# rcelha/rio-rs

Measured on AMD Instinct MI355X. Metric: placement decisions/sec + achieved HBM GB/s, 10M objects x 1 024 nodes, higher is better.
Workload: dtype u32; 1 GPU; config 3: 10000000 objects x 1024 nodes, Zipf(1.1) load, cap 1.25x; a stream of committed ticks that starts from the cold table (all pending); objects_per_gpu=10000000, nodes=1024, parallelism=rows sharded x1

## Files before the change

### include/rio_gpu_placement_debug.h

```cpp
#ifndef RIO_GPU_PLACEMENT_DEBUG_H
#define RIO_GPU_PLACEMENT_DEBUG_H

#include "rio_gpu_placement.h"

#ifdef __cplusplus
extern "C" {
#endif

int rio_gp_debug_set_compact(rio_gp_t* h, int mode);
uint64_t rio_gp_debug_chained_scans(rio_gp_t* h);
int rio_gp_debug_set_speculate(rio_gp_t* h, int speculate);
int rio_gp_debug_set_node_index(rio_gp_t* h, uint32_t tile_rows);
int rio_gp_debug_node_index_geometry(rio_gp_t* h, const uint64_t* node_bitmap, uint32_t* out4);
void rio_gp_debug_set_scan_nt(int mode);
void rio_gp_debug_set_part_shift(int shift);
uint64_t rio_gp_debug_wave_row_lo(uint64_t n_objects, uint32_t n_nodes, uint32_t wave, uint32_t* n_waves);
int rio_gp_debug_ktrace(rio_gp_t* h, int enable, int table, uint64_t* out2048);
int rio_gp_debug_stream_probe(rio_gp_t* h, int mode, int reps, float* ms);

#ifdef __cplusplus
}
#endif
#endif
```

### rio-rs_amd/csrc/placement_kernels.h

```cpp
#pragma once
#include <hip/hip_runtime.h>
#include <stdint.h>

namespace riogp {

typedef uint32_t u32;
typedef unsigned long long u64;

constexpr u32 kNone = 0xFFFFFFFFu;
constexpr u32 kSpillMark = 0xFFFFFFFEu;
constexpr u32 kSkipMark = 0xFFFFFFFDu;
constexpr u32 kAffInactive = 0xFFFFFFFEu;
constexpr u32 kFlagReplaced = 0x10u;
constexpr u32 kNoCut = 0xFFFFFFFFu;

constexpr int kWaves = 16;
constexpr int kBlock = kWaves * 64;
constexpr int kTile = 256;
constexpr u32 kMaxBlocks = 256;
constexpr u32 kMaxSubs = 256;
constexpr int kMidBatch = 16384;
constexpr int kReqBatch = 131072;
constexpr int kSmallBatch = 256;

struct Plan {
    u64 n;
    u64 tiles;
    u64 tq;
    u64 div_magic;
    u32 tr;
    u32 nw;
    u32 G;
    u32 sub;
    u32 subs;
    u32 m;
    u32 mwords;
    u32 trace;
    u32 sa;
    u64 mark;
    const u32* wcnt;
    u32* alive_dst;
};
Plan make_plan(u64 n, u32 m, u32 max_blocks);
// ... 21 lines not shown
    u64* H;
    u64* partial;
    u64* blkstat;
    u64* wsp_sum[2];
    u32* wsp_cnt[2];
    u64* bsp_sum[2];
    u32* bsp_cnt[2];
    u64* used_kept;
    u64* used_cur;
    u64* claim_tot;
    u32* cutblk;
    u64* budget;
    u64* admpre;
    u32* cutidx;
    u32* forced_bits;
    u64* rank_base;
    const u64* pending_global;
    const u64* run_if = nullptr;
    u64* RP;
    u64* R;
    u64* D;
    const u64* used_snap;
    u64* Tg = nullptr;
    DevStats* stats;
    FxRows fx;
};
constexpr u32 kFillRounds = 8;

struct PackOut {
    u32* idx;
    u32* load;
    u32* aff;
    u32* next;
    u32* wcnt;
};

struct Table {
    const u32* cur;
    const u32* load;
    const u32* aff;
    u32* next;
    const u32* pk_idx = nullptr;
    u32* real_next = nullptr;
    bool none_prewritten = false;
    const uint2* vrec = nullptr;
    bool prewritten = false;
// ... 18 lines not shown
    u64* rows = nullptr;
};

bool scan_chain_fits(u32 m);

void launch_scan(const Plan& p, const Table& t, const NodeTab& nt, const SolveBufs& b, bool virt, bool all_alive,
                 hipStream_t s, hipEvent_t e0 = nullptr, hipEvent_t e1 = nullptr, const PackOut* pack = nullptr,
                 const ScanChain* chain = nullptr);
void launch_resolve(const Plan& p, const NodeTab& nt, const SolveBufs& b, u64* host_partial, hipStream_t s,
                    hipEvent_t e0 = nullptr, hipEvent_t e1 = nullptr, const PackOut* search = nullptr,
                    u64* fold_into = nullptr, u32 fold_rounds = 0, const u64* kept_from = nullptr, const u64* fold_from = nullptr);
bool inc_scan_fits(u32 m);
void launch_inc_scan(const Plan& p, u32* assign, const u32* load, const u32* aff, const NodeTab& nt, const SolveBufs& b,
                     const PackOut& pack, hipStream_t s);
Plan rebal_plan(const Plan& p);
u64 rebal_rows(u64 n);
void launch_rebal(const Plan& p, const Plan& pv, const PackOut& src, const NodeTab& nt, const PackOut& dst, const SolveBufs& b,
                  hipStream_t s);
unsigned resolve_blocks(u32 m);
void set_scan_nt(int mode);
void launch_cut_find(const Plan& p, const Table& t, const NodeTab& nt, const SolveBufs& b, bool virt, hipStream_t s,
                     bool have_cutblk);
void launch_fill(const Plan& p, const Table& t, const NodeTab& nt, const SolveBufs& b, bool virt, bool apply, bool fill,
                 int round, bool last, hipStream_t s, const PackOut* pack = nullptr);
bool fill_can_pack(u32 m);
bool cut_apply_fits(u32 m);
void launch_cut_apply(const Plan& p, const Table& t, const NodeTab& nt, const SolveBufs& b, const PackOut& pk, const PackOut& ul,
                      u64* Tg, bool pack, bool all_alive, hipStream_t s);
void launch_used_fold(u64* used, const u64* D, u32 m, u32 rounds, hipStream_t s);
#ifdef RIO_GP_LAB
int ktrace_enable(int on);
int ktrace_read(int table, u64* out );
float sync_probe(int mode, int reps, hipStream_t s);
float stream_probe(int mode, const u32* a, const u32* b, const u32* c, u32* o, u64 n, int reps, hipStream_t s,
                   hipEvent_t e0, hipEvent_t e1);
#endif

struct SmallInline { u32 a[4]; u32 b[4]; };
void launch_lookup_small(const u32* assign, u64 n_obj, const u32* idx, u32 n, u32* out, DevStats* st, hipStream_t s,
                         u32* done, u32 seq, const SmallInline* inl = nullptr);
void launch_lookup(const u32* assign, u64 n_obj, const u32* idx, u64 n, u32* out, DevStats* st, hipStream_t s,
                   u32* done = nullptr, u32 seq = 0, unsigned int* ticket = nullptr);
void launch_update(u32* assign, u64 n_obj, u32 m, const u32* idx, const u32* node, u64 n, u32* pos_scratch,
                   DevStats* st, hipStream_t s, u32* aff_life = nullptr, unsigned int* ticket = nullptr, u32* done = nullptr,
                   u32 seq = 0, u64* used = nullptr, const u32* load = nullptr);
void launch_update_small(u32* assign, const u32* idx, const u32* node, u32 n, hipStream_t s, u32* aff_life = nullptr,
                         u32* done = nullptr, u32 seq = 0, const SmallInline* inl = nullptr, u64* used = nullptr,
// ... 186 lines not shown
```

### rio-rs_amd/csrc/placement_kernels.hip

```cpp
#include "placement_kernels.h"
#include <algorithm>
#include <cstdlib>

#include <hip/hip_ext.h>

namespace riogp {


template <int CTRL>
__device__ __forceinline__ u64 dpp64(u64 v) {
    const u32 lo = (u32)__builtin_amdgcn_update_dpp(0, (int)(u32)v, CTRL, 0xf, 0xf, false);
    const u32 hi = (u32)__builtin_amdgcn_update_dpp(0, (int)(u32)(v >> 32), CTRL, 0xf, 0xf, false);
    return ((u64)hi << 32) | lo;
}
template <int CTRL>
__device__ __forceinline__ u32 dpp32(u32 v) {
    return (u32)__builtin_amdgcn_update_dpp(0, (int)v, CTRL, 0xf, 0xf, false);
}
__device__ __forceinline__ u64 shfl_up64(u64 v, int d) {
    u32 lo = __shfl_up((u32)v, d, 64), hi = __shfl_up((u32)(v >> 32), d, 64);
    return ((u64)hi << 32) | lo;
}
__device__ __forceinline__ u64 shfl_xor64(u64 v, int d) {
    u32 lo = __shfl_xor((u32)v, d, 64), hi = __shfl_xor((u32)(v >> 32), d, 64);
// ... 1723 lines not shown
        rk[q] = 0;
        if (q < per && cls[q] < 0x100u)
            rk[q] = (u32)ctot[cls[q]] + (u32)tab[((size_t)cls[q] * per + q) * kWaves + wave] + pos[q];
    }
    RIOGP_KT(p, 4, 4);
    return all;
}


struct FillArgs {
    const u32* cur; const u32* load; const u32* aff; u32* next;
    const u32* alive_bits;
    Plan p;
    const u32* cutidx; const u32* forced_bits;
    const u64* cap; const u64* Uread; const u64* D; u64* Uadd; u32 round;
    const u64* wsp_sum_in; const u32* wsp_cnt_in; u64* wsp_sum_out; u32* wsp_cnt_out;
    const u64* bsp_sum_in; const u32* bsp_cnt_in; u64* bsp_sum_out; u32* bsp_cnt_out;
    const u64* R; const u64* RP; u32 ng;
    int last;
    DevStats* stats;
    const u32* pk_idx; u32* real_next;
    const u64* rank_base; const u64* pending_global;
    const u64* run_if;
    FxRows fx;
    PackOut pko;
};

__host__ __device__ __forceinline__ size_t fill_lds_x(u32 m, u32 mwords, bool pack) {
    const size_t a = (size_t)m * sizeof(u64);
    const size_t b = (size_t)((m + 3) & ~3u) * sizeof(u32) + (size_t)((mwords + 3) & ~3u) * sizeof(u32) +
                     (pack ? (size_t)kWaves * 2 * kStageCap * sizeof(u32) : 0);
    const size_t c = rank_tab_bytes(m);
    const size_t x = a > b ? a : b;
    return ((x > c ? x : c) + 15) & ~(size_t)15;
}
__host__ __device__ __forceinline__ size_t fill_lds_off_ord(u32 m) { return 512 + (((size_t)(m + 1) * sizeof(u64) + 15) & ~(size_t)15); }
__host__ __device__ __forceinline__ size_t fill_lds_off_x(u32 m) { return fill_lds_off_ord(m) + (((size_t)m * sizeof(unsigned short) + 15) & ~(size_t)15); }

template <bool VIRT, bool APPLY, bool FILL, bool PACK>
__global__ __launch_bounds__(kBlock) void k_fill(const FillArgs a) {
    extern __shared__ __attribute__((aligned(16))) unsigned char smem[];
    const Plan& p = a.p;
    const u32 m = p.m;
    const bool sa_ = p.sa != 0;
    u64* red = reinterpret_cast<u64*>(smem);
    u64* part = reinterpret_cast<u64*>(smem + 128);
// ... 39 lines not shown
    if (FILL) {
#pragma unroll
        for (u32 q = 0; q < 8; ++q) fr[q] = 0;
        pgv = a.pending_global ? *a.pending_global : 0ull;
        rbv = a.rank_base ? *a.rank_base : 0ull;
#pragma unroll
        for (u32 q = 0; q < 8; ++q) {
            if (q < per) {
                const u32 j = tid + q * kBlock, jj = j < m ? j : m - 1;
                u64 u = a.Uread[jj];
                if (a.D)
                    for (u32 r = 0; r < a.round; ++r) u += a.D[(size_t)r * m + jj];
                const u64 c = a.cap[jj];
                const bool al = bit_of(a.alive_bits, jj);
                fr[q] = (j < m && al && c > u) ? c - u : 0ull;
            }
        }
    }
    const u32 bt = (u32)tid < G ? (u32)tid : G - 1;
    const u64 bv = a.bsp_sum_in[bt] + ((APPLY && FILL) ? a.R[bt] : 0ull);
    const u64 rpv = (APPLY && FILL) ? a.RP[(size_t)((u32)tid < a.ng ? (u32)tid : a.ng - 1) * G + blockIdx.x] : 0ull;
    const u32 bc = a.bsp_cnt_in[bt];
    const u64 pw = a.wsp_sum_in[w0 + (tid & (kWaves - 1))];
    u64 wstart = wave_row_lo(p, gw), wend = wave_row_lo(p, gw + 1);
    if (wend > p.n) wend = p.n;
    if (wstart > wend) wstart = wend;
    if (p.wcnt && wstart + wc < wend) wend = wstart + wc;
    u64 bstart = wstart, bend = wend;
    if (FILL && !APPLY && pc == 0) bend = bstart;
    u32 own_cnt = pc;
    const u64 rs = (wstart < wend ? wstart : 0ull) + (u64)lane * 4;
    uint4 cvn = make_uint4(0, 0, 0, 0), avn = cvn, lvn = cvn, nvn = cvn, ivn = cvn;
    const bool scat = a.pk_idx != nullptr;
    if (APPLY) {
        cvn = *reinterpret_cast<const uint4*>(a.cur + rs);
        avn = *reinterpret_cast<const uint4*>(a.aff + rs);
        lvn = *reinterpret_cast<const uint4*>(a.load + rs);
        if (FILL && !PACK) ivn = *reinterpret_cast<const uint4*>((scat ? a.pk_idx : a.load) + rs);
    } else {
        const u64 rb = (bstart < bend ? bstart : 0ull) + (u64)lane * 4;
        nvn = *reinterpret_cast<const uint4*>(a.next + rb);
        lvn = *reinterpret_cast<const uint4*>(a.load + rb);
        ivn = *reinterpret_cast<const uint4*>((scat ? a.pk_idx : a.load) + rb);
    }

    if (APPLY && !FILL) {
// ... 1 lines not shown
        if (PACK && ncut == 0 && a.forced_bits == nullptr && a.bsp_cnt_in[blockIdx.x] == 0) {
            if (lane == 0) a.pko.wcnt[gw] = 0;
            return;
        }
    }
    if (tid < 16) red[tid] = 0;
    if (FILL)
        for (u32 k = tid; k < (u32)(rank_tab_bytes(m) / 4); k += kBlock) reinterpret_cast<u32*>(X)[k] = 0;
    __syncthreads();
    u64 blk_base = 0;
    if (FILL) {
        u64 sb = ((u32)tid < G && (u32)tid < blockIdx.x) ? bv : 0ull;
        if (APPLY && (u32)tid < a.ng) sb += rpv;
        u32 c = (u32)tid < G ? bc : 0u;
        sb = wave_sum(sb);
        c = wave_sum32(c);
        if (lane == 0 && (sb | c)) { atomicAdd(&red[0], sb); atomicAdd(&red[1], (u64)c); }
        __syncthreads();
        const bool pending = a.pending_global ? (pgv != 0) : (red[1] != 0 || (APPLY && (ncut != 0 || a.forced_bits != nullptr)));
        if (!pending) {
            if (lane == 0) {
                a.wsp_sum_out[gw] = 0;
                a.wsp_cnt_out[gw] = 0;
                if (PACK) a.pko.wcnt[gw] = 0;
            }
            if (tid == 0) { a.bsp_sum_out[blockIdx.x] = 0; a.bsp_cnt_out[blockIdx.x] = 0; }
            if (a.last && a.fx.dev && a.fx.seq && tid < 8)
                a.fx.host[(size_t)blockIdx.x * 8 + tid] = tid == 7 ? a.fx.seq : a.fx.dev[(size_t)blockIdx.x * 8 + tid];
            return;
        }
        if (!a.fx.dev && blockIdx.x == 0 && tid == 0) atomicAdd(&a.stats->rounds_run, 1ull);
        blk_base = red[0] + rbv;
        RIOGP_KT(p, kt, 1);
    }

    if (FILL) {
        u32 rk[8];
        cnt = rank_by_class(reinterpret_cast<unsigned short*>(X), per, fr, rk, p);
#pragma unroll
        for (u32 q = 0; q < 8; ++q)
            if (q < per && fr[q] != 0) { C[rk[q] + 1] = fr[q]; ord[rk[q]] = (unsigned short)(tid + q * kBlock); }
        __syncthreads();
        RIOGP_KT(p, 4, 5);
        u64 fk[8];
        u64 loc = 0;
#pragma unroll
// ... 147 lines not shown
    u32* const bnext = PACK ? a.pko.next : a.next;
    const u32* const bload = PACK ? a.pko.load : a.load;
    const u32* const bidx = PACK ? a.pko.idx : a.pk_idx;
    for (u32 k = tid; k < m; k += kBlock) adm[k] = 0;
    __syncthreads();
    RIOGP_KT(p, kt, 4);
    u64 run = blk_base;
    for (int w = 0; w < wave; ++w) run += wsum[w];
    const u64 F = C[cnt];
    u64 rem_sum = 0, pl_sum = 0;
    u32 rem_cnt = 0, pl_cnt = 0;
    u32 lo_run = 0;
    if (cnt) {
        u32 lo = 0, hi = cnt;
        while (hi - lo > 1) {
            const u32 mid = lo + ((hi - lo) >> 1);
            if (C[mid] <= run) lo = mid; else hi = mid;
        }
        lo_run = lo;
    }
    const int last = a.last;
    const bool quiet_tail = !last || (bscat && last == 2);
    const u64 run0 = run;
    for (u64 it = bstart; it < bend; it += kTile) {
        if (quiet_tail && (cnt == 0 || run >= F)) {
            const u32 seen = wave_sum32(pl_cnt + rem_cnt);
            if (lane == 0) { rem_sum += wsum[wave] - (run - run0); rem_cnt += own_cnt - seen; }
            break;
        }
        const u64 i0 = it + (u64)lane * 4;
        const uint4 nv = nvn, lv = lvn, iv = ivn;
        const u64 pit = it + kTile < bend ? it + kTile : it;
        nvn = *reinterpret_cast<const uint4*>(bnext + pit + (u64)lane * 4);
        lvn = *reinterpret_cast<const uint4*>(bload + pit + (u64)lane * 4);
        if (bscat) ivn = *reinterpret_cast<const uint4*>(bidx + pit + (u64)lane * 4);
        const bool mk0 = i0 + 0 < bend && nv.x == kSpillMark, mk1 = i0 + 1 < bend && nv.y == kSpillMark;
        const bool mk2 = i0 + 2 < bend && nv.z == kSpillMark, mk3 = i0 + 3 < bend && nv.w == kSpillMark;
        if (!__ballot(mk0 | mk1 | mk2 | mk3)) continue;
        const u64 l0 = mk0 ? lv.x : 0, l1 = mk1 ? lv.y : 0;
        const u64 l2 = mk2 ? lv.z : 0, l3 = mk3 ? lv.w : 0;
        const u64 lsum = l0 + l1 + l2 + l3;
        if (cnt == 0 || run >= F) {
            rem_sum += lsum;
            rem_cnt += (u32)mk0 + (u32)mk1 + (u32)mk2 + (u32)mk3;
            if (last) {
                uint4 ov = nv;
                ov.x = mk0 ? kNone : ov.x; ov.y = mk1 ? kNone : ov.y; ov.z = mk2 ? kNone : ov.z; ov.w = mk3 ? kNone : ov.w;
                *reinterpret_cast<uint4*>(bnext + i0) = ov;
                if (bscat && last == 1) {
                    if (mk0) a.real_next[iv.x] = kNone;
                    if (mk1) a.real_next[iv.y] = kNone;
                    if (mk2) a.real_next[iv.z] = kNone;
                    if (mk3) a.real_next[iv.w] = kNone;
                }
            }
            continue;
        }
        const u64 inc = wave_incl_scan(lsum, lane);
        u64 Q = run + (inc - lsum);
        const u64 run_end = run + shfl64(inc, 63);
        u32 hi_run = lo_run;
        {
            u32 step = 1;
            while (hi_run + step < cnt && C[hi_run + step] <= run_end) { hi_run += step; step <<= 1; }
            u32 top = hi_run + step < cnt ? hi_run + step : cnt;
            while (top - hi_run > 1) {
                const u32 mid = hi_run + ((top - hi_run) >> 1);
                if (C[mid] <= run_end) hi_run = mid; else top = mid;
            }
        }
        uint4 ov = nv;
        uint4 wv = make_uint4(kKeepVal, kKeepVal, kKeepVal, kKeepVal);
        if (hi_run == lo_run && run_end <= C[lo_run + 1]) {
            const u32 nd0 = (u32)ord[lo_run];
            ov.x = mk0 ? nd0 : ov.x; ov.y = mk1 ? nd0 : ov.y; ov.z = mk2 ? nd0 : ov.z; ov.w = mk3 ? nd0 : ov.w;
            pl_sum += lsum;
            pl_cnt += (u32)mk0 + (u32)mk1 + (u32)mk2 + (u32)mk3;
            if (lane == 0) atomicAdd(&adm[nd0], run_end - run);
            *reinterpret_cast<uint4*>(bnext + i0) = ov;
            if (bscat) {
                if (mk0) a.real_next[iv.x] = nd0;
                if (mk1) a.real_next[iv.y] = nd0;
                if (mk2) a.real_next[iv.z] = nd0;
                if (mk3) a.real_next[iv.w] = nd0;
            }
            run = run_end;
            continue;
        }
        u32 pn[4] = {kNone, kNone, kNone, kNone};
        u64 pll[4] = {0, 0, 0, 0};
#define RIOGP_ROW(MK, L, E, OUT, WOUT)                                            \
        if (MK) {                                                                 \
            u32 nd = kNone;                                                       \
            if (Q < F) {                                                          \
                u32 lo = lo_run, hi = hi_run + 1;                                 \
                while (hi - lo > 1) {                                             \
                    const u32 mid = lo + ((hi - lo) >> 1);                        \
                    if (C[mid] <= Q) lo = mid; else hi = mid;                     \
                }                                                                 \
                if (Q + L <= C[lo + 1]) nd = (u32)ord[lo];                        \
            }                                                                     \
            if (nd != kNone) {                                                    \
                OUT = nd;                                                         \
                WOUT = nd;                                                        \
                pn[E] = nd; pll[E] = (u64)L;                                      \
                pl_sum += L; ++pl_cnt;                                            \
            } else {                                                              \
                if (last) {                                                       \
                    OUT = kNone;                                                  \
                    if (last == 1) WOUT = kNone;   \
                }                                                                 \
                rem_sum += L; ++rem_cnt;                                          \
            }                                                                     \
            Q += L;                                                               \
        }
        RIOGP_ROW(mk0, l0, 0, ov.x, wv.x)
        RIOGP_ROW(mk1, l1, 1, ov.y, wv.y)
        RIOGP_ROW(mk2, l2, 2, ov.z, wv.z)
        RIOGP_ROW(mk3, l3, 3, ov.w, wv.w)
#undef RIOGP_ROW
        {
            const u32 n0 = pn[0] != kNone ? pn[0] : pn[1] != kNone ? pn[1] : pn[2] != kNone ? pn[2] : pn[3];
            const u64 pmask = __ballot(n0 != kNone);
            if (pmask) {
                const u32 nd0 = (u32)__builtin_amdgcn_readlane((int)n0, __ffsll((long long)pmask) - 1);
                const bool odd = (pn[0] != kNone && pn[0] != nd0) | (pn[1] != kNone && pn[1] != nd0) |
                                 (pn[2] != kNone && pn[2] != nd0) | (pn[3] != kNone && pn[3] != nd0);
                if (!__ballot(odd)) {
                    const u64 tot = wave_sum(pll[0] + pll[1] + pll[2] + pll[3]);
                    if (lane == 0) atomicAdd(&adm[nd0], tot);
                } else {
#pragma unroll
                    for (int e = 0; e < 4; ++e)
                        if (pn[e] != kNone) atomicAdd(&adm[pn[e]], pll[e]);
                }
            }
        }
        if ((ov.x != nv.x) | (ov.y != nv.y) | (ov.z != nv.z) | (ov.w != nv.w)) *reinterpret_cast<uint4*>(bnext + i0) = ov;
        if (bscat) {
            if (wv.x != kKeepVal) a.real_next[iv.x] = wv.x;
            if (wv.y != kKeepVal) a.real_next[iv.y] = wv.y;
            if (wv.z != kKeepVal) a.real_next[iv.z] = wv.z;
            if (wv.w != kKeepVal) a.real_next[iv.w] = wv.w;
        }
        run = run_end;
        lo_run = hi_run;
    }
    RIOGP_KT(p, kt, 5);
    rem_sum = wave_sum(rem_sum);
    rem_cnt = wave_sum32(rem_cnt);
    pl_sum = wave_sum(pl_sum);
    pl_cnt = wave_sum32(pl_cnt);
    if (lane == 0) {
        a.wsp_sum_out[gw] = rem_sum;
        a.wsp_cnt_out[gw] = rem_cnt;
        if (pl_cnt) { atomicAdd(&red[2], (u64)pl_cnt); atomicAdd(&red[3], pl_sum); }
        if (rem_cnt) { atomicAdd(&red[4], rem_sum); atomicAdd(&red[5], (u64)rem_cnt); }
    }
    __syncthreads();
    RIOGP_KT(p, kt, 6);
    if (tid == 0) { a.bsp_sum_out[blockIdx.x] = red[4]; a.bsp_cnt_out[blockIdx.x] = (u32)red[5]; }
    for (u32 k = tid; k < m; k += kBlock)
        if (adm[k]) atomicAdd(&a.Uadd[k], adm[k]);
    if (a.fx.dev) {
        if (tid < 8) {
            u64* r = a.fx.dev + (size_t)blockIdx.x * 8;
            const u64 add = tid == 0 ? red[6] : tid == 1 ? red[7] : tid == 2 ? red[2] : tid == 3 ? red[3]
                          : (tid == 4 && last) ? red[5] : (tid == 5 && last) ? red[4]
                          : (tid == 6 && blockIdx.x == 0) ? 1ull : 0ull;
            const u64 v = (tid == 7 && last && a.fx.seq) ? a.fx.seq : r[tid] + add;
            r[tid] = v;
            a.fx.host[(size_t)blockIdx.x * 8 + tid] = v;
        }
    } else if (tid == 0) {
        if (APPLY && red[6]) { atomicAdd(&a.stats->rejected, red[6]); atomicAdd(&a.stats->load_rejected, red[7]); }
        if (red[2]) { atomicAdd(&a.stats->spilled, red[2]); atomicAdd(&a.stats->load_spilled, red[3]); }
        if (last && red[5]) { atomicAdd(&a.stats->unplaced, red[5]); atomicAdd(&a.stats->load_unplaced, red[4]); }
    }
// ... 2376 lines not shown
}

void launch_cut_find(const Plan& p, const Table& t, const NodeTab& nt, const SolveBufs& b, bool virt, hipStream_t s,
                     bool have_cutblk) {
    const unsigned gcb = (p.m + kCbNodes - 1) / kCbNodes;
    if (!have_cutblk)
        hipLaunchKernelGGL(k_cutblk, dim3(gcb ? gcb : 1), dim3(256), 0, s, b.H, p, nt.cap, nt.alive_bits, b.used_kept,
                           b.claim_tot, b.cutblk, b.budget, b.admpre, b.stats);
    u32 tcap = 0;
    const size_t ldsf = cut_find_lds(p, &tcap);
    u64* R = have_cutblk ? b.R : nullptr;
    if (virt)
        hipLaunchKernelGGL(k_cut_find<true>, dim3(kCutFindGrid), dim3(kBlock), ldsf, s, t.cur, t.load, t.aff, nt.alive_bits, p,
                           b.cutblk, b.budget, b.admpre, b.used_kept, b.forced_bits, b.cutidx, b.used_cur, b.stats, tcap, R);
    else
        hipLaunchKernelGGL(k_cut_find<false>, dim3(kCutFindGrid), dim3(kBlock), ldsf, s, t.cur, t.load, t.aff, nt.alive_bits, p,
                           b.cutblk, b.budget, b.admpre, b.used_kept, b.forced_bits, b.cutidx, b.used_cur, b.stats, tcap, R);
}

static size_t fill_lds_bytes(u32 m, u32 mwords, bool pack) { return fill_lds_off_x(m) + fill_lds_x(m, mwords, pack) + 16; }
bool fill_can_pack(u32 m) { return fill_lds_bytes(m, (m + 31) / 32, true) <= (size_t)160 * 1024; }

void launch_fill(const Plan& p, const Table& t, const NodeTab& nt, const SolveBufs& b, bool virt, bool apply, bool fill,
                 int round, bool last, hipStream_t s, const PackOut* pack) {
    const int in = (apply ? 0 : (round & 1)), out = fill ? (in ^ 1) : 0;
    FillArgs a;
    a.cur = t.cur; a.load = t.load; a.aff = t.aff; a.next = t.next;
    a.alive_bits = nt.alive_bits;
    a.p = p;
    a.cutidx = b.cutidx; a.forced_bits = b.forced_bits;
    a.cap = nt.cap; a.round = (u32)round;
    if (b.D) { a.Uread = b.used_cur; a.D = b.D; a.Uadd = b.D + (size_t)round * p.m; }
    else { a.Uread = b.used_snap ? b.used_snap : b.used_cur; a.D = nullptr; a.Uadd = b.used_cur; }
    a.wsp_sum_in = b.wsp_sum[in]; a.wsp_cnt_in = b.wsp_cnt[in]; a.wsp_sum_out = b.wsp_sum[out]; a.wsp_cnt_out = b.wsp_cnt[out];
    a.bsp_sum_in = b.bsp_sum[in]; a.bsp_cnt_in = b.bsp_cnt[in]; a.bsp_sum_out = b.bsp_sum[out]; a.bsp_cnt_out = b.bsp_cnt[out];
    a.R = b.R; a.RP = b.RP; a.ng = resolve_blocks(p.m);
    a.last = last ? ((t.none_prewritten || pack) ? 2 : 1) : 0;
    a.stats = b.stats;
    a.pk_idx = t.pk_idx; a.real_next = pack ? t.next : t.real_next;
    a.rank_base = b.rank_base; a.pending_global = b.pending_global; a.run_if = b.run_if;
    a.fx = b.fx;
    a.pko = pack ? *pack : PackOut{nullptr, nullptr, nullptr, nullptr, nullptr};
    const size_t lds = fill_lds_bytes(p.m, p.mwords, pack != nullptr);
    if (apply && fill) {
        if (virt) hipLaunchKernelGGL((k_fill<true, true, true, false>), dim3(p.G), dim3(kBlock), lds, s, a);
        else if (pack) hipLaunchKernelGGL((k_fill<false, true, true, true>), dim3(p.G), dim3(kBlock), lds, s, a);
        else hipLaunchKernelGGL((k_fill<false, true, true, false>), dim3(p.G), dim3(kBlock), lds, s, a);
    } else if (fill) {
        hipLaunchKernelGGL((k_fill<false, false, true, false>), dim3(p.G), dim3(kBlock), lds, s, a);
    } else {
        if (virt) hipLaunchKernelGGL((k_fill<true, true, false, false>), dim3(p.G), dim3(kBlock), lds, s, a);
        else hipLaunchKernelGGL((k_fill<false, true, false, false>), dim3(p.G), dim3(kBlock), lds, s, a);
    }
}

bool cut_apply_fits(u32 m) { return m >= 1 && ca_lds_bytes(m, (m + 31) / 32) <= (size_t)150 * 1024; }
void launch_cut_apply(const Plan& p, const Table& t, const NodeTab& nt, const SolveBufs& b, const PackOut& pk, const PackOut& ul,
                      u64* Tg, bool pack, bool all_alive, hipStream_t s) {
    CutApplyArgs a;
    a.cur = t.cur; a.load = t.load; a.aff = t.aff; a.next = t.next;
    a.alive_bits = nt.alive_bits;
    a.p = p;
    a.p.wcnt = nullptr;
// ... 1496 lines not shown
```

### rio-rs_amd/csrc/rio_gp_capi.hip

```cpp
#include <hip/hip_runtime.h>
#include <dlfcn.h>

#include <cstdio>
#include <cstdlib>
#include <cstring>
#include <chrono>
#include <algorithm>
#include <atomic>
#include <mutex>
#include <string>
#include <vector>

#include "../../include/rio_gpu_placement.h"
#ifdef RIO_GP_LAB
#include "../../include/rio_gpu_placement_debug.h"
#endif
#include "placement_kernels.h"

using namespace riogp;

namespace {

thread_local std::string g_create_error;
struct RioGpNcclId { char internal[128]; };
// ... 137 lines not shown
    u64* Tg = nullptr;
    Plan vplan{};
    int cutpack_mode = 0;
    bool ca_now = false;
    hipStream_t scan2 = nullptr;
    u32* chain_flags = nullptr;
    u32 *h_chain_err = nullptr, *d_chain_err = nullptr;
    u32 chain_seq = 0, chain_prev = 0, chain_pos = 0;
    hipEvent_t ev_run = nullptr;
    u64 overlap_min_rows = (u64)1 << 18;
    hipEvent_t ev_join = nullptr;
    u64* used_ring = nullptr;
    size_t used_slot_words = 0;
    u32 used_base = 0;
    u64* solve_used = nullptr;
    int chain_diag = 0;
    bool chain_ok = false;
    u64 chain_total = 0;
    int chain_mode = 0;
    int cutapply_mode = 0;
    u64 last_fix_rows = 0;
    bool last_fix_valid = false;
    int spec_mode = 0;
    int part_mode = 0;
    bool last_slow = false;
    u32* h_cs = nullptr;
    u32* d_cs = nullptr;
    size_t cs_words = 0;
    u64* cs_cnt = nullptr;
    unsigned int* cs_ticket = nullptr;
    u32* h_small = nullptr;
    u32* d_small = nullptr;
    u64 wait_seq = 1;
    u32* h_mid = nullptr;
    u32* d_mid = nullptr;
    unsigned int* mid_ticket = nullptr;
    u32* h_req = nullptr;
    u32* d_req = nullptr;
    u32* pp_bad = nullptr;
    u64* pp_claim = nullptr;
    bool pp_last_slow = false;
    DevBuf rq[4];
    void* pp_stage = nullptr;
    u32 small_seq = 0;
    DevBuf vt[4], stage[4];
    DevBuf vrec;
// ... 160 lines not shown
    (void)chain_owner(h).compare_exchange_strong(me, nullptr, std::memory_order_acq_rel);
}
void chain_join(rio_gp* h) {
    if (!h->chain_prev) return;
    (void)hipSetDevice(h->device);
    if (h->chain_pos >= 2 &&
        (hipEventRecord(h->ev_join, h->scan2) != hipSuccess || hipStreamWaitEvent(h->stream, h->ev_join, 0) != hipSuccess)) {
        (void)hipGetLastError();
        (void)hipStreamSynchronize(h->scan2);
    }
    chain_end(h);
}
struct Locked {
    std::unique_lock<std::mutex> l;
    explicit Locked(rio_gp* h, bool join = true) : l(h->mu) { if (join) chain_join(h); }
};
bool use_cut_apply(rio_gp* h, u32 m) { return h->cutapply_mode != 2 && !h->sb.forced_bits && cut_apply_fits(m); }
bool cut_apply_for(rio_gp* h, bool cutpack) {
    return use_cut_apply(h, h->m) && (h->cutapply_mode == 1 || (cutpack && h->rounds >= 1 && fill_can_pack(h->m)));
}

void enqueue_slow(rio_gp* h, const Plan& p, const Table& t, const NodeTab& nt, bool virt, bool searched, bool cutpack = false) {
    cutpack = cutpack && !virt && !p.wcnt && h->rounds >= 1 && fill_can_pack(p.m);
    if (!virt && !searched && !p.wcnt && h->ca_now) {
        launch_cut_apply(p, t, nt, h->sb, h->pk, h->pk2, h->Tg, cutpack, h->all_alive, h->stream);
        if (cutpack) {
            Plan pp = p;
            pp.wcnt = h->pk.wcnt;
            Table vt{h->pos , h->pk.load, h->pk.aff, h->pk.next};
            vt.pk_idx = h->pk.idx;
            vt.real_next = t.next;
            vt.none_prewritten = true;
            for (u32 r = 0; r < h->rounds; ++r) launch_fill(pp, vt, nt, h->sb, true, false, true, (int)r, r + 1 == h->rounds, h->stream);
        } else {
            for (u32 r = 0; r < h->rounds; ++r) launch_fill(p, t, nt, h->sb, false, false, true, (int)r, r + 1 == h->rounds, h->stream);
        }
        return;
    }
    if (!searched) launch_cut_find(p, t, nt, h->sb, virt, h->stream, true);
    launch_fill(p, t, nt, h->sb, virt, true, true, 0, h->rounds == 1, h->stream, cutpack ? &h->pk : nullptr);
    if (cutpack) {
        Plan pp = p;
        pp.wcnt = h->pk.wcnt;
        Table vt{h->pos , h->pk.load, h->pk.aff, h->pk.next};
        vt.pk_idx = h->pk.idx;
        vt.real_next = t.next;
        vt.none_prewritten = true;
        for (u32 r = 1; r < h->rounds; ++r) launch_fill(pp, vt, nt, h->sb, true, false, true, (int)r, r + 1 == h->rounds, h->stream);
        return;
    }
    for (u32 r = 1; r < h->rounds; ++r) launch_fill(p, t, nt, h->sb, virt, false, true, (int)r, r + 1 == h->rounds, h->stream);
}

const u64* parts_src(rio_gp* h) { return h->parts ? h->parts : h->D; }
void fold_used(rio_gp* h) {
    if (!h->used_parts) return;
    launch_used_fold(h->used, parts_src(h), h->m, h->parts_rounds, h->stream);
    h->used_parts = false;
}
void enqueue_scan_resolve(rio_gp* h, const Table& t, const NodeTab& nt, bool compact, u64* host_rows, int inc = 0) {
    h->sb.D = h->D;
    h->solve_used_D = h->sb.D != nullptr;
    h->inc_now = inc;
    h->solve_inplace = inc != 0;
    const PackOut& pkx = inc == 2 ? h->pk2 : h->pk;
    h->vplan = h->plan;
    SolveBufs rb = h->sb;
    h->ca_now = h->ca_now && !compact && !inc;
    if (h->ca_now) { rb.R = nullptr; rb.RP = nullptr; rb.Tg = h->Tg; }
    if (inc) {
        launch_inc_scan(h->plan, h->assign[h->cur], h->load, h->aff, nt, h->sb, h->pk, h->stream);
        h->vplan = rebal_plan(h->plan);
        launch_rebal(h->plan, h->vplan, h->pk, nt, h->pk2, h->sb, h->stream);
    } else {
// ... 428 lines not shown
    }
    h->chain_ok = h->scan2 && scan_chain_fits((u32)h->cap_nodes);
#ifdef RIO_GP_LAB
    if (const char* e = getenv("RIO_GP_CHAIN_DIAG")) h->chain_diag = atoi(e);
    if (const char* e = getenv("RIO_GP_OVERLAP_MIN_ROWS")) h->overlap_min_rows = strtoull(e, nullptr, 10);
#endif
    const size_t R = h->cap_rows, M = h->cap_nodes, W = (size_t)kMaxBlocks * kWaves;
    const size_t R2 = std::max((size_t)rebal_rows(h->cap_obj) + 8 * kTile, R);
#define A(ptr, cnt) if ((rc = dalloc(h, &(ptr), (cnt))) != RIO_GP_OK) return bail(rc)
    A(h->assign[0], R); A(h->assign[1], R); A(h->load, R); A(h->aff, R); A(h->pos, R2);
    h->used_slot_words = (h->chain_ok ? (size_t)kChainReps : 1) * M;
    A(h->cap, M); A(h->used_ring, kUsedRing * h->used_slot_words); A(h->alive_bits, (M + 31) / 32 + 4); A(h->dead_bits, (M + 31) / 32 + 4);
    A(h->alive_bytes, M);
    A(h->sb.H, (size_t)((M + 7) / 8) * kMaxBlocks * 16); A(h->sb.blkstat, (size_t)kMaxBlocks * 4);
    A(h->sb.partial, (size_t)resolve_blocks((u32)M) * 8 + 8);
    A(h->sb.wsp_sum[0], W); A(h->sb.wsp_sum[1], W); A(h->sb.wsp_cnt[0], W); A(h->sb.wsp_cnt[1], W);
    A(h->sb.bsp_sum[0], (size_t)kMaxBlocks); A(h->sb.bsp_sum[1], (size_t)kMaxBlocks); A(h->sb.bsp_cnt[0], (size_t)kMaxBlocks); A(h->sb.bsp_cnt[1], (size_t)kMaxBlocks);
    A(h->sb.used_kept, M); A(h->sb.claim_tot, M); A(h->sb.cutblk, M); A(h->sb.budget, M);
    A(h->sb.admpre, M); A(h->sb.cutidx, M); A(h->dstats, 1); A(h->fx_dev, (size_t)kMaxBlocks * 8);
    A(h->sb.R, (size_t)kMaxBlocks); A(h->sb.RP, (size_t)kMaxBlocks * resolve_blocks((u32)M)); A(h->D, (size_t)kFillRounds * M);
    A(h->pk.idx, R); A(h->pk.load, R); A(h->pk.aff, R); A(h->pk.next, R); A(h->pk.wcnt, W);
    A(h->pk2.idx, R2); A(h->pk2.load, R2); A(h->pk2.aff, R2); A(h->pk2.next, R2); A(h->pk2.wcnt, W);
    A(h->Tg, M * kWaves);
    A(h->chain_flags, W);
    A(h->sh_lkept, M); A(h->sh_lclaim, M); A(h->sh_lcur, M); A(h->sh_lcutblk, M); A(h->sh_lcutidx, M);
    A(h->sh_gprev, M); A(h->sh_gfinal, M); A(h->sh_rank_base, 2); A(h->sh_verdict, 8); A(h->sh_forced, (M + 31) / 32 + 4);
#undef A
    h->used = h->used_ring;
    h->sb.used_cur = h->used_ring + h->used_slot_words;
    h->sb.stats = h->dstats;
    if (hipHostMalloc(reinterpret_cast<void**>(&h->h_stats), sizeof(DevStats) * kRing, hipHostMallocMapped) !=
        hipSuccess) {
        h->err = "hipHostMalloc failed";
        return bail(RIO_GP_ENOMEM);
    }
    if (hipHostMalloc(reinterpret_cast<void**>(&h->h_chain_err), 64, hipHostMallocMapped) != hipSuccess ||
        hipHostGetDevicePointer(reinterpret_cast<void**>(&h->d_chain_err), h->h_chain_err, 0) != hipSuccess) {
        h->err = "hipHostMalloc(chain error word) failed";
        return bail(RIO_GP_ENOMEM);
    }
    memset(h->h_chain_err, 0, 64);
    h->slot_rows = std::max<size_t>(resolve_blocks(h->cap_nodes), kMaxBlocks);
    if (hipHostMalloc(reinterpret_cast<void**>(&h->h_slots), (size_t)2 * kRing * h->slot_rows * 8 * sizeof(u64),
                      hipHostMallocMapped) != hipSuccess ||
        hipHostMalloc(reinterpret_cast<void**>(&h->h_fx), (size_t)(1 + kRing) * kMaxBlocks * 8 * sizeof(u64), hipHostMallocMapped) != hipSuccess ||
        hipHostGetDevicePointer(reinterpret_cast<void**>(&h->d_fx), h->h_fx, 0) != hipSuccess ||
// ... 2364 lines not shown
}

uint64_t rio_gp_debug_chained_scans(rio_gp_t* h) {
    if (!h) return 0;
    Locked g(h);
    return h->chain_total;
}

int rio_gp_debug_set_node_index(rio_gp_t* h, uint32_t tile_rows) {
    if (!h) return RIO_GP_EINVAL;
    Locked g(h);
    h->ni_force_tile = tile_rows;
    return RIO_GP_OK;
}
int rio_gp_debug_node_index_geometry(rio_gp_t* h, const uint64_t* node_bitmap, uint32_t* out4) {
    if (!h || !out4) return RIO_GP_EINVAL;
    Locked g(h);
    u32 s = 0;
    for (u32 j = 0; j < h->m; ++j) s += !node_bitmap || ((node_bitmap[j >> 6] >> (j & 63)) & 1ull);
    const NiPlan p = ni_plan(h->n, h->m, s, 0, 0, h->ni_force_tile);
    out4[0] = (u32)p.T; out4[1] = p.nt; out4[2] = p.cb; out4[3] = p.W;
    return RIO_GP_OK;
}
int rio_gp_debug_set_speculate(rio_gp_t* h, int speculate) {
    if (!h || speculate < 0 || speculate > 2) return RIO_GP_EINVAL;
    Locked g(h);
    h->spec_mode = speculate;
    return RIO_GP_OK;
}

int rio_gp_debug_ktrace(rio_gp_t* h, int enable, int table, uint64_t* out2048) {
    if (!h) return RIO_GP_EINVAL;
    Locked g(h);
    HIPCHK(h, hipSetDevice(h->device));
    HIPCHK(h, hipStreamSynchronize(h->stream));
    if (out2048 && ktrace_read(table, reinterpret_cast<u64*>(out2048)) != 0) return fail(h, RIO_GP_EUPSTREAM, "ktrace read failed");
    ktrace_enable(enable);
    return RIO_GP_OK;
}

int rio_gp_debug_stream_probe(rio_gp_t* h, int mode, int reps, float* ms) {
    if (!h || !ms || reps < 1) return RIO_GP_EINVAL;
    Locked g(h);
    HIPCHK(h, hipSetDevice(h->device));
    if (mode >= 20 && mode <= 23) {
        *ms = sync_probe(mode, reps, h->stream);
// ... 39 lines not shown
```

### rio-rs_amd/rio_gp.py

```python
import ctypes as C
import os
import subprocess

import numpy as np

_DIR = os.path.dirname(os.path.abspath(__file__))
LIB_PATH = os.path.join(_DIR, "librio_gp.so")
NONE = 0xFFFFFFFF
CAP_INF = 0xFFFFFFFFFFFFFFFF
AFF_INACTIVE = 0xFFFFFFFE
CFG_ROW_LIFECYCLE = 1
CFG_REF_SELF_ASSIGN = 2
OP_CFG_NO_HOST_SHADOW = 8
OP_CFG_LIVE_FIRST_TOUCH = 4
FLAG_LOCAL, FLAG_REDIRECT, FLAG_PLACED, FLAG_SPILLED, FLAG_UNPLACED = range(5)
FLAG_REPLACED = 0x10
FLAG_MASK = 0x0F
CHANGES_PEEK = 1
NODE_GONE = 0xFFFFFFFC
OK, EINVAL, EUPSTREAM, ENODEV, ENOMEM, ERANGE, EAGAIN = range(7)
ABI_VERSION = 2

LAB_PATH = os.path.join(_DIR, "librio_gp_lab.so")
SOURCES = [os.path.join(_DIR, "csrc", f) for f in ("placement_kernels.hip", "rio_gp_capi.hip", "gpu_object_placement.cpp")]
# ... 155 lines not shown
        L.rio_gp_solve_profiled.argtypes = [_vp, C.POINTER(C.c_float), C.POINTER(C.c_float)]
        L.rio_gp_set_object_attrs.argtypes = [_vp, C.c_uint64, _vp, _vp, _vp]
        L.rio_gp_get_objects.argtypes = [_vp, C.c_uint64, _vp, _vp]
        L.rio_gp_set_num_objects.argtypes = [_vp, C.c_uint64]
        L.rio_gp_place_pending_dev.argtypes = [_vp, C.c_uint64, _vp, _vp, _vp, _vp]
        L.rio_gp_mixed_batch.argtypes = [_vp, C.POINTER(Mixed)]
        for nm in ("rio_gp_rows_on_nodes", "rio_gp_rows_on_nodes_dev"):
            getattr(L, nm).argtypes = [_vp, _vp, _vp, _vp, C.c_uint64, C.POINTER(C.c_uint64)]
        for nm in ("rio_gp_rebalance", "rio_gp_rebalance_dev"):
            getattr(L, nm).argtypes = [_vp, C.POINTER(RebalanceCfg), C.POINTER(RebalanceStats), _vp, _vp, _vp, C.c_uint64,
                                       C.POINTER(C.c_uint64)]
        for nm in ("rio_gp_changes", "rio_gp_changes_dev"):
            getattr(L, nm).argtypes = [_vp, C.c_uint32, _vp, _vp, _vp, C.c_uint64, C.POINTER(C.c_uint64)]
        L.rio_gp_changes_reset.argtypes = [_vp]
        L.rio_gp_remap_nodes.argtypes = [_vp, C.c_uint32, _vp, C.POINTER(C.c_uint64)]
        if lab:
            L.rio_gp_debug_set_scan_nt.argtypes = [C.c_int]
            L.rio_gp_debug_set_scan_nt.restype = None
            L.rio_gp_debug_set_part_shift.argtypes = [C.c_int]
            L.rio_gp_debug_set_part_shift.restype = None
            L.rio_gp_debug_stream_probe.argtypes = [_vp, C.c_int, C.c_int, C.POINTER(C.c_float)]
            L.rio_gp_debug_set_compact.argtypes = [_vp, C.c_int]
            L.rio_gp_debug_set_speculate.argtypes = [_vp, C.c_int]
            L.rio_gp_debug_chained_scans.argtypes = [_vp]
            L.rio_gp_debug_chained_scans.restype = C.c_uint64
            L.rio_gp_debug_ktrace.argtypes = [_vp, C.c_int, C.c_int, C.POINTER(C.c_uint64)]
            L.rio_gp_debug_wave_row_lo.argtypes = [C.c_uint64, C.c_uint32, C.c_uint32, C.POINTER(C.c_uint32)]
            L.rio_gp_debug_wave_row_lo.restype = C.c_uint64
            L.rio_gp_debug_set_node_index.argtypes = [_vp, C.c_uint32]
            L.rio_gp_debug_node_index_geometry.argtypes = [_vp, _vp, _vp]
        L.rio_gp_timer_begin.argtypes = [_vp]
        L.rio_gp_timer_stop.argtypes = [_vp]
        L.rio_gp_timer_end.argtypes = [_vp, C.POINTER(C.c_float)]
        _libs[lab] = L
    return _libs[lab]


def _ptr(a):
    return None if a is None else a.ctypes.data_as(_vp)


def _u32(a):
    return None if a is None else np.ascontiguousarray(a, dtype=np.uint32)


class GpuPlacement:
# ... 363 lines not shown
        modes = {"auto": 0, "always": 1, "never": 2}
        incs = {"auto": 0, "always": 1, "never": 2}
        self._chk(self._L.rio_gp_debug_set_compact(self._h, modes.get(mode, mode) | (0 if partitioned_crud else 16) |
                                                   (modes.get(cut_pack, cut_pack) << 5) | (incs.get(inc, inc) << 7) |
                                                   (modes.get(cut_apply, cut_apply) << 9) | (0 if chain else 4096)))

    def chained_scans(self):
        self._need_lab()
        return int(self._L.rio_gp_debug_chained_scans(self._h))

    def set_node_index(self, tile_rows=0):
        self._need_lab()
        self._chk(self._L.rio_gp_debug_set_node_index(self._h, int(tile_rows)))

    def node_index_geometry(self, nodes=None):
        self._need_lab()
        out = np.zeros(4, np.uint32)
        self._chk(self._L.rio_gp_debug_node_index_geometry(self._h, _ptr(self._node_bitmap(nodes)), _ptr(out)))
        return tuple(int(x) for x in out)

    def set_speculate(self, speculate="auto"):
        self._need_lab()
        self._chk(self._L.rio_gp_debug_set_speculate(self._h, {"auto": 0, "always": 1, "never": 2}.get(speculate, speculate)))

    def timer_begin(self):
        self._chk(self._L.rio_gp_timer_begin(self._h))

    def timer_stop(self):
        self._chk(self._L.rio_gp_timer_stop(self._h))

    def timer_end(self):
        ms = C.c_float(0)
        self._chk(self._L.rio_gp_timer_end(self._h, C.byref(ms)))
        return float(ms.value)



class OpCfg(C.Structure):
    _fields_ = [("struct_size", C.c_uint32), ("device", C.c_int32), ("max_objects", C.c_uint64),
                ("max_nodes", C.c_uint32), ("spill_rounds", C.c_uint32), ("flags", C.c_uint32),
                ("collect_ns", C.c_uint32)]


_op_ready = False


# ... 283 lines not shown
```

Before: 427.4 billion decisions/s.

## Record per-wave leftover rows in fill rounds to skip rescanning tiles

Fill rounds can now record the spilled (stay) rows of each wave, up to 64 per wave, as index/load pairs in double-buffered per-wave lists. The next round reads those lists and places the entries directly with a single wave scan and binary search, instead of walking the wave's whole row range again. Waves whose spill count exceeds the cap fall back to the full walk. This adds extra global writes and branching to every fill round in exchange for shorter later rounds. It is on by default, and a debug toggle can disable it.

```diff
diff --git a/include/rio_gpu_placement_debug.h b/include/rio_gpu_placement_debug.h
--- a/include/rio_gpu_placement_debug.h
+++ b/include/rio_gpu_placement_debug.h
@@ -10,6 +10,7 @@
 int rio_gp_debug_set_compact(rio_gp_t* h, int mode);
 uint64_t rio_gp_debug_chained_scans(rio_gp_t* h);
 int rio_gp_debug_set_speculate(rio_gp_t* h, int speculate);
+int rio_gp_debug_set_leftover(rio_gp_t* h, int mode);
 int rio_gp_debug_set_node_index(rio_gp_t* h, uint32_t tile_rows);
 int rio_gp_debug_node_index_geometry(rio_gp_t* h, const uint64_t* node_bitmap, uint32_t* out4);
 void rio_gp_debug_set_scan_nt(int mode);
diff --git a/rio-rs_amd/csrc/placement_kernels.h b/rio-rs_amd/csrc/placement_kernels.h
--- a/rio-rs_amd/csrc/placement_kernels.h
+++ b/rio-rs_amd/csrc/placement_kernels.h
@@ -19,6 +19,8 @@
 constexpr int kTile = 256;
 constexpr u32 kMaxBlocks = 256;
 constexpr u32 kMaxSubs = 256;
+constexpr u32 kLeftCap = 64;
+constexpr u32 kLeftWalk = 0xFFFFFFFFu;
 constexpr int kMidBatch = 16384;
 constexpr int kReqBatch = 131072;
 constexpr int kSmallBatch = 256;
@@ -86,6 +88,8 @@
     u64* D;
     const u64* used_snap;
     u64* Tg = nullptr;
+    u64* left[2] = {nullptr, nullptr};
+    u32* left_cnt[2] = {nullptr, nullptr};
     DevStats* stats;
     FxRows fx;
 };
@@ -150,7 +154,8 @@
 void launch_cut_find(const Plan& p, const Table& t, const NodeTab& nt, const SolveBufs& b, bool virt, hipStream_t s,
                      bool have_cutblk);
 void launch_fill(const Plan& p, const Table& t, const NodeTab& nt, const SolveBufs& b, bool virt, bool apply, bool fill,
-                 int round, bool last, hipStream_t s, const PackOut* pack = nullptr);
+                 int round, bool last, hipStream_t s, const PackOut* pack = nullptr, int lists = 0);
+constexpr int kLeftRead = 1, kLeftWrite = 2;
 bool fill_can_pack(u32 m);
 bool cut_apply_fits(u32 m);
 void launch_cut_apply(const Plan& p, const Table& t, const NodeTab& nt, const SolveBufs& b, const PackOut& pk, const PackOut& ul,
diff --git a/rio-rs_amd/csrc/placement_kernels.hip b/rio-rs_amd/csrc/placement_kernels.hip
--- a/rio-rs_amd/csrc/placement_kernels.hip
+++ b/rio-rs_amd/csrc/placement_kernels.hip
@@ -1769,6 +1769,7 @@
     const u32* pk_idx; u32* real_next;
     const u64* rank_base; const u64* pending_global;
     const u64* run_if;
+    const u64* left_in; const u32* left_cnt_in; u64* left_out; u32* left_cnt_out;
     FxRows fx;
     PackOut pko;
 };
@@ -1854,6 +1855,12 @@
     const u64 rpv = (APPLY && FILL) ? a.RP[(size_t)((u32)tid < a.ng ? (u32)tid : a.ng - 1) * G + blockIdx.x] : 0ull;
     const u32 bc = a.bsp_cnt_in[bt];
     const u64 pw = a.wsp_sum_in[w0 + (tid & (kWaves - 1))];
+    u32 lc = kLeftWalk;
+    u64 ent = 0;
+    if (FILL && !APPLY) {
+        lc = *(a.left_in ? a.left_cnt_in + gw : a.wsp_cnt_in + gw);
+        ent = *(a.left_in ? a.left_in + gw * kLeftCap + lane : a.wsp_sum_in + gw);
+    }
     u64 wstart = wave_row_lo(p, gw), wend = wave_row_lo(p, gw + 1);
     if (wend > p.n) wend = p.n;
     if (wstart > wend) wstart = wend;
@@ -1901,6 +1908,7 @@
             if (lane == 0) {
                 a.wsp_sum_out[gw] = 0;
                 a.wsp_cnt_out[gw] = 0;
+                if (a.left_out) a.left_cnt_out[gw] = 0;
                 if (PACK) a.pko.wcnt[gw] = 0;
             }
             if (tid == 0) { a.bsp_sum_out[blockIdx.x] = 0; a.bsp_cnt_out[blockIdx.x] = 0; }
@@ -2094,10 +2102,61 @@
     const int last = a.last;
     const bool quiet_tail = !last || (bscat && last == 2);
     const u64 run0 = run;
+    u32 lcur = 0;
+    u64* const lout = a.left_out ? a.left_out + gw * kLeftCap : nullptr;
+    if (FILL && !APPLY && a.left_in && lc - 1u < kLeftCap && lc == pc && !(quiet_tail && (cnt == 0 || run >= F))) {
+        const bool on = (u32)lane < lc;
+        const u32 pos = on ? (u32)ent : 0u;
+        const u64 L = on ? ent >> 32 : 0ull;
+        const u32 ridx = bscat ? bidx[pos] : 0u;
+        const u64 inc = wave_incl_scan(L, lane);
+        const u64 Q = run + (inc - L);
+        const u64 run_end = run + shfl64(inc, 63);
+        u32 hi_run = lo_run;
+        {
+            u32 step = 1;
+            while (hi_run + step < cnt && C[hi_run + step] <= run_end) { hi_run += step; step <<= 1; }
+            u32 top = hi_run + step < cnt ? hi_run + step : cnt;
+            while (top - hi_run > 1) {
+                const u32 mid = hi_run + ((top - hi_run) >> 1);
+                if (C[mid] <= run_end) hi_run = mid; else top = mid;
+            }
+        }
+        u32 nd = kNone;
+        if (on && Q < F) {
+            u32 lo = lo_run, hi = hi_run + 1;
+            while (hi - lo > 1) {
+                const u32 mid = lo + ((hi - lo) >> 1);
+                if (C[mid] <= Q) lo = mid; else hi = mid;
+            }
+            if (Q + L <= C[lo + 1]) nd = (u32)ord[lo];
+        }
+        const bool stay = on && nd == kNone;
+        if (on && !stay) {
+            bnext[pos] = nd;
+            if (bscat) a.real_next[ridx] = nd;
+            atomicAdd(&adm[nd], L);
+            pl_sum += L; ++pl_cnt;
+        }
+        if (stay) {
+            if (last) {
+                bnext[pos] = kNone;
+                if (bscat && last == 1) a.real_next[ridx] = kNone;
+            }
+            rem_sum += L; ++rem_cnt;
+        }
+        const u64 sb = __ballot(stay);
+        if (lout && sb) {
+            if (stay) lout[__popcll(sb & ((1ull << lane) - 1ull))] = ent;
+            lcur = (u32)__popcll(sb);
+        }
+        bend = bstart;
+    }
     for (u64 it = bstart; it < bend; it += kTile) {
         if (quiet_tail && (cnt == 0 || run >= F)) {
             const u32 seen = wave_sum32(pl_cnt + rem_cnt);
             if (lane == 0) { rem_sum += wsum[wave] - (run - run0); rem_cnt += own_cnt - seen; }
+            lcur = kLeftWalk;
             break;
         }
         const u64 i0 = it + (u64)lane * 4;
@@ -2115,6 +2174,7 @@
         if (cnt == 0 || run >= F) {
             rem_sum += lsum;
             rem_cnt += (u32)mk0 + (u32)mk1 + (u32)mk2 + (u32)mk3;
+            lcur = kLeftWalk;
             if (last) {
                 uint4 ov = nv;
                 ov.x = mk0 ? kNone : ov.x; ov.y = mk1 ? kNone : ov.y; ov.z = mk2 ? kNone : ov.z; ov.w = mk3 ? kNone : ov.w;
@@ -2161,6 +2221,7 @@
         }
         u32 pn[4] = {kNone, kNone, kNone, kNone};
         u64 pll[4] = {0, 0, 0, 0};
+        u32 stay = 0;
 #define RIOGP_ROW(MK, L, E, OUT, WOUT)                                            \
         if (MK) {                                                                 \
             u32 nd = kNone;                                                       \
@@ -2182,6 +2243,7 @@
                     OUT = kNone;                                                  \
                     if (last == 1) WOUT = kNone;   \
                 }                                                                 \
+                stay |= 1u << E;                                                  \
                 rem_sum += L; ++rem_cnt;                                          \
             }                                                                     \
             Q += L;                                                               \
@@ -2215,6 +2277,24 @@
             if (wv.z != kKeepVal) a.real_next[iv.z] = wv.z;
             if (wv.w != kKeepVal) a.real_next[iv.w] = wv.w;
         }
+        if (lout && lcur != kLeftWalk) {
+            const u64 sb = __ballot(stay != 0);
+            if (sb) {
+                const u32 mine = (u32)__popc(stay);
+                const u32 sinc = (u32)wave_incl_scan((u64)mine, lane);
+                const u32 tot = (u32)__builtin_amdgcn_readlane((int)sinc, 63);
+                if (lcur + tot > kLeftCap) {
+                    lcur = kLeftWalk;
+                } else {
+                    u32 e = lcur + sinc - mine;
+                    if (stay & 1u) lout[e++] = (u64)(u32)(i0 + 0) | l0 << 32;
+                    if (stay & 2u) lout[e++] = (u64)(u32)(i0 + 1) | l1 << 32;
+                    if (stay & 4u) lout[e++] = (u64)(u32)(i0 + 2) | l2 << 32;
+                    if (stay & 8u) lout[e++] = (u64)(u32)(i0 + 3) | l3 << 32;
+                    lcur += tot;
+                }
+            }
+        }
         run = run_end;
         lo_run = hi_run;
     }
@@ -2226,6 +2306,7 @@
     if (lane == 0) {
         a.wsp_sum_out[gw] = rem_sum;
         a.wsp_cnt_out[gw] = rem_cnt;
+        if (lout) a.left_cnt_out[gw] = lcur;
         if (pl_cnt) { atomicAdd(&red[2], (u64)pl_cnt); atomicAdd(&red[3], pl_sum); }
         if (rem_cnt) { atomicAdd(&red[4], rem_sum); atomicAdd(&red[5], (u64)rem_cnt); }
     }
@@ -4648,7 +4729,7 @@
 bool fill_can_pack(u32 m) { return fill_lds_bytes(m, (m + 31) / 32, true) <= (size_t)160 * 1024; }
 
 void launch_fill(const Plan& p, const Table& t, const NodeTab& nt, const SolveBufs& b, bool virt, bool apply, bool fill,
-                 int round, bool last, hipStream_t s, const PackOut* pack) {
+                 int round, bool last, hipStream_t s, const PackOut* pack, int lists) {
     const int in = (apply ? 0 : (round & 1)), out = fill ? (in ^ 1) : 0;
     FillArgs a;
     a.cur = t.cur; a.load = t.load; a.aff = t.aff; a.next = t.next;
@@ -4665,6 +4746,9 @@
     a.stats = b.stats;
     a.pk_idx = t.pk_idx; a.real_next = pack ? t.next : t.real_next;
     a.rank_base = b.rank_base; a.pending_global = b.pending_global; a.run_if = b.run_if;
+    const bool lrd = fill && !apply && (lists & kLeftRead) && b.left[in], lwr = fill && !last && (lists & kLeftWrite) && b.left[out];
+    a.left_in = lrd ? b.left[in] : nullptr; a.left_cnt_in = lrd ? b.left_cnt[in] : nullptr;
+    a.left_out = lwr ? b.left[out] : nullptr; a.left_cnt_out = lwr ? b.left_cnt[out] : nullptr;
     a.fx = b.fx;
     a.pko = pack ? *pack : PackOut{nullptr, nullptr, nullptr, nullptr, nullptr};
     const size_t lds = fill_lds_bytes(p.m, p.mwords, pack != nullptr);
diff --git a/rio-rs_amd/csrc/rio_gp_capi.hip b/rio-rs_amd/csrc/rio_gp_capi.hip
--- a/rio-rs_amd/csrc/rio_gp_capi.hip
+++ b/rio-rs_amd/csrc/rio_gp_capi.hip
@@ -183,6 +183,7 @@
     u64 last_fix_rows = 0;
     bool last_fix_valid = false;
     int spec_mode = 0;
+    int left_mode = 0;
     int part_mode = 0;
     bool last_slow = false;
     u32* h_cs = nullptr;
@@ -389,6 +390,7 @@
 
 void enqueue_slow(rio_gp* h, const Plan& p, const Table& t, const NodeTab& nt, bool virt, bool searched, bool cutpack = false) {
     cutpack = cutpack && !virt && !p.wcnt && h->rounds >= 1 && fill_can_pack(p.m);
+    const int lw = h->left_mode == 2 ? 0 : kLeftWrite, lrw = h->left_mode == 2 ? 0 : (kLeftRead | kLeftWrite);
     if (!virt && !searched && !p.wcnt && h->ca_now) {
         launch_cut_apply(p, t, nt, h->sb, h->pk, h->pk2, h->Tg, cutpack, h->all_alive, h->stream);
         if (cutpack) {
@@ -398,14 +400,16 @@
             vt.pk_idx = h->pk.idx;
             vt.real_next = t.next;
             vt.none_prewritten = true;
-            for (u32 r = 0; r < h->rounds; ++r) launch_fill(pp, vt, nt, h->sb, true, false, true, (int)r, r + 1 == h->rounds, h->stream);
+            for (u32 r = 0; r < h->rounds; ++r)
+                launch_fill(pp, vt, nt, h->sb, true, false, true, (int)r, r + 1 == h->rounds, h->stream, nullptr, r ? lrw : lw);
         } else {
-            for (u32 r = 0; r < h->rounds; ++r) launch_fill(p, t, nt, h->sb, false, false, true, (int)r, r + 1 == h->rounds, h->stream);
+            for (u32 r = 0; r < h->rounds; ++r)
+                launch_fill(p, t, nt, h->sb, false, false, true, (int)r, r + 1 == h->rounds, h->stream, nullptr, r ? lrw : lw);
         }
         return;
     }
     if (!searched) launch_cut_find(p, t, nt, h->sb, virt, h->stream, true);
-    launch_fill(p, t, nt, h->sb, virt, true, true, 0, h->rounds == 1, h->stream, cutpack ? &h->pk : nullptr);
+    launch_fill(p, t, nt, h->sb, virt, true, true, 0, h->rounds == 1, h->stream, cutpack ? &h->pk : nullptr, lw);
     if (cutpack) {
         Plan pp = p;
         pp.wcnt = h->pk.wcnt;
@@ -413,10 +417,11 @@
         vt.pk_idx = h->pk.idx;
         vt.real_next = t.next;
         vt.none_prewritten = true;
-        for (u32 r = 1; r < h->rounds; ++r) launch_fill(pp, vt, nt, h->sb, true, false, true, (int)r, r + 1 == h->rounds, h->stream);
+        for (u32 r = 1; r < h->rounds; ++r)
+            launch_fill(pp, vt, nt, h->sb, true, false, true, (int)r, r + 1 == h->rounds, h->stream, nullptr, lrw);
         return;
     }
-    for (u32 r = 1; r < h->rounds; ++r) launch_fill(p, t, nt, h->sb, virt, false, true, (int)r, r + 1 == h->rounds, h->stream);
+    for (u32 r = 1; r < h->rounds; ++r) launch_fill(p, t, nt, h->sb, virt, false, true, (int)r, r + 1 == h->rounds, h->stream, nullptr, lrw);
 }
 
 const u64* parts_src(rio_gp* h) { return h->parts ? h->parts : h->D; }
@@ -891,6 +896,7 @@
     A(h->pk.idx, R); A(h->pk.load, R); A(h->pk.aff, R); A(h->pk.next, R); A(h->pk.wcnt, W);
     A(h->pk2.idx, R2); A(h->pk2.load, R2); A(h->pk2.aff, R2); A(h->pk2.next, R2); A(h->pk2.wcnt, W);
     A(h->Tg, M * kWaves);
+    A(h->sb.left[0], W * kLeftCap); A(h->sb.left[1], W * kLeftCap); A(h->sb.left_cnt[0], W); A(h->sb.left_cnt[1], W);
     A(h->chain_flags, W);
     A(h->sh_lkept, M); A(h->sh_lclaim, M); A(h->sh_lcur, M); A(h->sh_lcutblk, M); A(h->sh_lcutidx, M);
     A(h->sh_gprev, M); A(h->sh_gfinal, M); A(h->sh_rank_base, 2); A(h->sh_verdict, 8); A(h->sh_forced, (M + 31) / 32 + 4);
@@ -3301,6 +3307,12 @@
     out4[0] = (u32)p.T; out4[1] = p.nt; out4[2] = p.cb; out4[3] = p.W;
     return RIO_GP_OK;
 }
+int rio_gp_debug_set_leftover(rio_gp_t* h, int mode) {
+    if (!h || (mode != 0 && mode != 2)) return RIO_GP_EINVAL;
+    Locked g(h);
+    h->left_mode = mode;
+    return RIO_GP_OK;
+}
 int rio_gp_debug_set_speculate(rio_gp_t* h, int speculate) {
     if (!h || speculate < 0 || speculate > 2) return RIO_GP_EINVAL;
     Locked g(h);
diff --git a/rio-rs_amd/rio_gp.py b/rio-rs_amd/rio_gp.py
--- a/rio-rs_amd/rio_gp.py
+++ b/rio-rs_amd/rio_gp.py
@@ -201,6 +201,7 @@
             L.rio_gp_debug_stream_probe.argtypes = [_vp, C.c_int, C.c_int, C.POINTER(C.c_float)]
             L.rio_gp_debug_set_compact.argtypes = [_vp, C.c_int]
             L.rio_gp_debug_set_speculate.argtypes = [_vp, C.c_int]
+            L.rio_gp_debug_set_leftover.argtypes = [_vp, C.c_int]
             L.rio_gp_debug_chained_scans.argtypes = [_vp]
             L.rio_gp_debug_chained_scans.restype = C.c_uint64
             L.rio_gp_debug_ktrace.argtypes = [_vp, C.c_int, C.c_int, C.POINTER(C.c_uint64)]
@@ -610,6 +611,10 @@
     def set_speculate(self, speculate="auto"):
         self._need_lab()
         self._chk(self._L.rio_gp_debug_set_speculate(self._h, {"auto": 0, "always": 1, "never": 2}.get(speculate, speculate)))
+
+    def set_leftover(self, on=True):
+        self._need_lab()
+        self._chk(self._L.rio_gp_debug_set_leftover(self._h, 0 if on else 2))
 
     def timer_begin(self):
         self._chk(self._L.rio_gp_timer_begin(self._h))
```

New measurement: 427.1 billion decisions/s. Within noise of the previous version (-0.1%).
